# JiehongLin/SAM-6D

Hardware: AMD Instinct MI355X
Metric: RGB-D frames/sec (SAM-6D per-frame hot path: SAM ViT-H encoder + ISM scoring + PEM) (higher is better)
Workload: dtype bf16 (SAM ViT-H: 87 % of the step) + f16 (PEM ViT-B feature extractor) + f32 (ISM scoring, PEM point transformer and pose solvers); 1 GPU; LM-O single object: 32 frames/step/GPU, 640x480 RGB-D -> 1024^2 SAM input, P=128 proposals x 42 templates (scored in groups of 8 frames), 1 instance/frame, 2048 pts (PEM batch 32); sam_frames_per_launch_group=16, pem_vit_dtype=fp16 (set by bench.py; the library default is fp32)

## Files before the change

include/sam6d_hip.h:

```cpp
#ifndef SAM6D_HIP_H
#define SAM6D_HIP_H

#include <stdint.h>

#ifdef __cplusplus
extern "C" {
#endif

#define S6D_OK 0
#define S6D_EINVAL (-1)
#define S6D_ELAUNCH (-2)
#define S6D_EUNSUPPORTED (-3)

#define S6D_ABI_VERSION 135
int s6d_version(void);
int s6d_set_persistent_grid_limit(int max_workgroups);
int s6d_set_gemm_wave_tile(int columns);
int s6d_set_gemm_mfma_shape(int rows);
int s6d_set_gemm_small_tile(int enable);
const char *s6d_strerror(int code);
const char *s6d_last_hip_error(void);


int s6d_fps_f32(const float *xyz, int B, int N, int M, float *tmp, int32_t *idx, void *stream);

int s6d_gather_points_f32(const float *points, const int32_t *idx, int B, int C, int N, int M,
                          float *out, void *stream);

int s6d_ball_query_f32(const float *new_xyz, const float *xyz, int B, int N, int M, float radius,
                       int nsample, int32_t *idx, void *stream);

int s6d_group_points_f32(const float *points, const int32_t *idx, int B, int C, int N, int M, int S,
                         float *out, void *stream);

int s6d_gather_rows_f32(const float *src, const int32_t *idx, int B, int N, int C, int M, float *out,
                        void *stream);

int s6d_segment_seq_sum_f32(const float *x, const int64_t *start, const int64_t *count, int P, int C, float *out,
                            void *stream);

int s6d_pem_sample_indices_f32(const float *keys, long key_stride, const int64_t *count, int P, int n_sample,
                               int64_t *idx, int32_t *overflow, void *stream);

int s6d_pem_mask_boxes_u8(const unsigned char *mask, const float *depth, int P, int H, int W, long min_points,
                          unsigned char *m, int64_t *cnt, unsigned char *ok, int64_t *box, void *stream);

int s6d_pem_compact_cloud_f32(const unsigned char *m, const float *depth, const int64_t *box, const unsigned char *ok, int P,
                              int H, int W, float fx, float fy, float cx, float cy, long cap, int32_t *choose, float *cloud,
                              int64_t *n, void *stream);
int s6d_pem_radius_filter_f32(const float *center, const double *limit, int P, long cap, int32_t *choose, float *cloud,
                              int64_t *n, void *stream);

int s6d_pem_crops_f32(const unsigned char *image, const unsigned char *m, const int64_t *kept, const int64_t *box, int M,
                      int H, int W, int S, int use_mask, const float *mean3_host, const float *std3_host, float *out,
                      void *stream);


int s6d_template_boxes_u8(const unsigned char *mask, int T, int H, int W, int64_t *cnt, int64_t *box, int64_t *tight,
                          void *stream);

int s6d_template_points_f32(const unsigned char *mask, const float *xyz_mm, const int64_t *box, int T, int H, int W, long cap,
                            int32_t *choose, float *pts, int64_t *n, void *stream);

int s6d_template_pem_crops_f32(const unsigned char *images, const unsigned char *mask, const int64_t *box, int T, int H, int W,
                               int S, int use_mask, const float *mean3_host, const float *std3_host, float *out, void *stream);

int s6d_template_ism_crops_f32(const unsigned char *images, const unsigned char *mask, const void *params, int T, int H, int W,
// ... 29 lines not shown


int s6d_mask_pack_u8(const uint8_t *masks, int N, long HW, uint64_t *packed, int32_t *area, void *stream);

int s6d_mask_pair_inter(const uint64_t *dpacked, int Nd, const uint64_t *gpacked, int Ng, long words, const int32_t *pairs, int P,
                        int32_t *inter, void *stream);

int s6d_box_pair_iou_f64(const double *dboxes, int Nd, const double *gboxes, int Ng, const int32_t *pairs, int P, double *iou,
                         void *stream);

#define S6D_COCO_MATCH_MAX_GT 64
int s6d_coco_match(const double *ious, const long *iou_off, const int32_t *groups, const double *det_area, const double *gt_area,
                   const uint8_t *gt_ignore, const double *params, int n_groups, int NT, int NA, long n_det, long n_gt, long n_iou,
                   int32_t *match, uint8_t *ignore, void *stream);


int s6d_rot_from_h_f32(const float *H, int n, float *R, void *stream);

int s6d_weighted_procrustes_f32(const float *src, const float *ref, const float *weights, int B, int N, float weight_thresh,
                                float eps, float *R, float *t, void *stream);

int s6d_pose_hypotheses_f32(const float *pts1, const float *pts2, const int32_t *pair, int B, int N1,
                            int N2, int n_hyp, float *R, float *t, float *dis, void *stream);

int s6d_cosine_similarity_f32(const float *f1, const float *f2, int B, int M1, int M2, int C, float temp, float *atten, void *stream);

int s6d_coarse_sample_f32(const float *atten, const float *rand_u, int B, int M1, int M2, int n_u, int32_t *pair, float *w1,
                          void *stream);

int s6d_smallest_k_f32(const float *dis, const float *Rs, const float *ts, int B, int n, int k, float *Rk, float *tk,
                       int32_t *idx, void *stream);

int s6d_hypothesis_select_f32(const float *dmin, const float *w1, const float *Rk, const float *tk, int B, int P, int N,
                              float *R, float *t, void *stream);

int s6d_min_dist_f32(const float *pts, const float *R, const float *t, const float *model, int B, int N,
                     int P, int Nm, float *dmin, void *stream);


int s6d_rpe_attention_f32(const float *q, const float *k, const float *v, const float *qt, const float *qb,
                          const float *embed, int B, int N, int C, int heads, float scale, float *out,
                          void *stream);

int s6d_rpe_attention_packed_f32(const float *proj, long ld, int q_off, int k_off, int v_off, int qt_off, int qb_off,
                                 const float *embed, int B, int N, int C, int heads, float scale, float *out, void *stream);
int s6d_rpe_attention_packed_e16_f32(const float *proj, long ld, int q_off, int k_off, int v_off, int qt_off, int qb_off,
                                     const void *embed_f16, int B, int N, int C, int heads, float scale, float *out, void *stream);
int s6d_rpe_attention_strided_e16_f32(const float *q, long ldq, const float *k, long ldk, const float *v, long ldv, const float *qt,
                                      const float *qb, const void *embed_f16, int B, int N, int C, int heads, float scale, float *out,
                                      void *stream);
int s6d_rpe_attention_strided_f32(const float *q, long ldq, const float *k, long ldk, const float *v, long ldv, const float *qt,
                                  const float *qb, const float *embed, int B, int N, int C, int heads, float scale, float *out,
                                  void *stream);


int s6d_win_attention_bf16(const void *qkv, const void *qkv_bias, const void *rel_h, const void *rel_w, int B,
                           int H, int W, int num_heads, int head_dim, int window, float scale, void *rel_scratch,
                           void *out, void *stream);
int s6d_win_attention_layout_bf16(const void *qkv, int head_major, const void *qkv_bias, const void *rel_h, const void *rel_w,
                                  int B, int H, int W, int num_heads, int head_dim, int window, float scale,
                                  void *rel_scratch, void *out, void *stream);
int s6d_win_attention_pad_rel_bf16(const void *rel_h, const void *rel_w, int H, int window, int head_dim, void *rel_padded, void *stream);
int s6d_win_attention_prepadded_bf16(const void *qkv, int head_major, const void *qkv_bias, const void *rel_padded, int B, int H, int W,
                                     int num_heads, int head_dim, int window, float scale, void *out, void *stream);
long s6d_win_attention_scratch_bytes(int H, int window, int head_dim);

int s6d_add_layernorm_bf16(const void *x, const void *delta, const float *gamma, const float *beta, float eps,
                           long rows, int C, void *x_out, void *y_out, void *stream);
int s6d_layernorm_bf16_f32(const void *x, const float *gamma, const float *beta, float eps, long rows, int C, float *y_f32,
                           void *stream);

int s6d_gemm_bf16(const void *A, long lda, const void *W, long ldw, const float *bias, void *C, long ldc, int M, int N,
                  int K, int epilogue, int max_blocks, void *stream);
int s6d_gemm_bf16_cblk(const void *A, long lda, const void *W, long ldw, const float *bias, void *C, long ldc, int M, int N, int K,
                       int epilogue, int col_block, int max_blocks, void *stream);
int s6d_gemm_f16(const void *A, long lda, const void *W, long ldw, const float *bias, void *C, long ldc, int M, int N, int K,
                 int epilogue, int max_blocks, void *stream);
int s6d_add_layernorm_f16(const void *x, const void *delta, const float *gamma, const float *beta, float eps, long rows, int C,
                          void *x_out, void *y_out, void *stream);
int s6d_seq_attention_f16(const void *qkv, int B, int N, int num_heads, int head_dim, float scale, void *out, void *stream);
int s6d_seq_attention_strided_bf16(const void *qkv, long tok_stride, long which_stride, long head_stride, int B, int N,
                                   int num_heads, int head_dim, float scale, void *out, void *stream);
int s6d_seq_attention_strided_f16(const void *qkv, long tok_stride, long which_stride, long head_stride, int B, int N,
                                  int num_heads, int head_dim, float scale, void *out, void *stream);

int s6d_gemm_bf16_res(const void *A, long lda, const void *W, long ldw, const float *bias, const void *R, long ldr,
                      float *stats_partial, void *C, long ldc, int M, int N, int K, int max_blocks, void *stream);
int s6d_ln_stats_finalize(const float *stats_partial, int groups, int group_size, long M, float eps, float *row_stats, void *stream);
int s6d_row_stats_bf16(const void *x, long ldx, long M, int C, float eps, float *row_stats, void *stream);
int s6d_gemm_bf16_lnfold(const void *A, long lda, const float *row_stats, const void *W, long ldw, const float *col_sums,
                         const float *bias, void *C, long ldc, int M, int N, int K, int gelu, int col_block, int max_blocks,
                         void *stream);

int s6d_gemm_fp8(const void *A, long lda, const unsigned char *a_scale, const void *W, long ldw, const unsigned char *w_scale,
                 const float *bias, void *C, long ldc, int M, int N, int K, int epilogue, int max_blocks, void *stream);
int s6d_gemm_fp8_gelu_mx(const void *A, long lda, const unsigned char *a_scale, const void *W, long ldw, const unsigned char *w_scale,
                         const float *bias, void *C8, long ldc, unsigned char *c_scale, int M, int N, int K, int max_blocks,
                         void *stream);
int s6d_gemm_fp8_mxa(const void *A, long lda, const unsigned char *a_mx, const void *W, long ldw, const unsigned char *w_scale,
                     const float *bias, void *C, long ldc, int M, int N, int K, int epilogue, int max_blocks, void *stream);
int s6d_layernorm_fp8(const void *x, const float *gamma, const float *beta, float eps, long rows, int C, void *y8,
                      unsigned char *yscale, void *stream);
int s6d_add_layernorm_fp8(const void *x, const void *delta, const float *gamma, const float *beta, float eps, long rows, int C,
                          void *x_out, void *y8, unsigned char *yscale, void *stream);


// ... 176 lines not shown
```

sam6d_amd/csrc/s6d_rpe.hip:

```cpp
#include "s6d_common.h"
#include "s6d_mem.h"

namespace s6d {

__device__ __forceinline__ float dot4(const float4 a, const float4 b) {
  return __builtin_fmaf(a.w, b.w, __builtin_fmaf(a.z, b.z, __builtin_fmaf(a.y, b.y, a.x * b.x)));
}

template <int WAVES, bool RPE, bool EH = false, int KEYS = 4>
__global__ __launch_bounds__(WAVES * 64) void rpe_attention_kernel(
    const float *__restrict__ q, const float *__restrict__ k, const float *__restrict__ v,
    const float *__restrict__ qt, const float *__restrict__ qb, const void *__restrict__ embedv,
    int B, int N, int M, float scale, float *__restrict__ out, long ldq, long ldk, long ldv, long qt_bs, long qt_rs, long qt_hs,
    long qb_bs, long qb_rs, long qb_hs) {
  S6D_DYN_LDS(smem);
  const int wave = threadIdx.x >> 6, lane = threadIdx.x & 63;
  const int Np = (M + 3) & ~3;
  float *sc = reinterpret_cast<float *>(smem) + (size_t)wave * 4 * Np;
  const long row = (long)blockIdx.x * WAVES + wave;
  if (row >= (long)B * N) return;
  const int b = (int)(row / N), n = (int)(row % N);
  const int g = lane >> 4;
  const int c4 = lane * 4;

  const float4 q4 = *reinterpret_cast<const float4 *>(q + row * ldq + c4);
  float4 t0 = make_float4(0.f, 0.f, 0.f, 0.f), t1 = t0, t2 = t0, t3 = t0;
  float qbg = 0.f;
  const float *erow = nullptr;
  const _Float16 *erow_h = nullptr;
  if (RPE) {
    const float *base = qt + (size_t)b * qt_bs + (size_t)n * qt_rs + c4;
    t0 = *reinterpret_cast<const float4 *>(base);
    t1 = *reinterpret_cast<const float4 *>(base + qt_hs);
    t2 = *reinterpret_cast<const float4 *>(base + 2 * qt_hs);
    t3 = *reinterpret_cast<const float4 *>(base + 3 * qt_hs);
    qbg = qb[(size_t)b * qb_bs + (size_t)n * qb_rs + (size_t)g * qb_hs];
    if (EH) erow_h = reinterpret_cast<const _Float16 *>(embedv) + (size_t)row * M * 256 + c4;
    else erow = reinterpret_cast<const float *>(embedv) + (size_t)row * M * 256 + c4;
  }
  const float *krow = k + (size_t)b * M * ldk + c4;
  const float *vrow = v + (size_t)b * M * ldv + c4;
  const bool hi32 = lane & 32, hi16 = lane & 16;

  const bool hi8 = lane & 8, hi4 = lane & 4;
  for (int m0 = 0; m0 < M; m0 += KEYS) {
    float4 k4[KEYS], e4[KEYS];
#pragma unroll
    for (int u = 0; u < KEYS; ++u) {
      const int m = min(m0 + u, M - 1);
      k4[u] = *reinterpret_cast<const float4 *>(krow + (size_t)m * ldk);
      if (RPE) {
        if (EH) {
          typedef __attribute__((ext_vector_type(4))) _Float16 h4;
          const h4 e = *reinterpret_cast<const h4 *>(erow_h + (size_t)m * 256);
          e4[u] = make_float4((float)e[0], (float)e[1], (float)e[2], (float)e[3]);
        } else {
          e4[u] = *reinterpret_cast<const float4 *>(erow + (size_t)m * 256);
        }
      }
    }
    float mine[KEYS];
#pragma unroll
    for (int u = 0; u < KEYS; ++u) {
      mine[u] = 0.f;
      if (RPE) {
        const float p0 = dot4(t0, e4[u]), p1 = dot4(t1, e4[u]), p2 = dot4(t2, e4[u]), p3 = dot4(t3, e4[u]);
        float ka = hi32 ? p2 : p0, kb = hi32 ? p3 : p1;
        const float sa = hi32 ? p0 : p2, sb = hi32 ? p1 : p3;
        ka += __shfl_xor(sa, 32);
        kb += __shfl_xor(sb, 32);
        mine[u] = hi16 ? kb : ka;
        const float send = hi16 ? ka : kb;
        mine[u] += __shfl_xor(send, 16);
      }
      mine[u] += dot4(q4, k4[u]);
    }
    float s;
    int mu = m0;
    bool writer;
    if (KEYS == 4) {
      float a0 = hi8 ? mine[1] : mine[0], a1 = hi8 ? mine[KEYS - 1] : mine[KEYS / 2];
      a0 += __shfl_xor(hi8 ? mine[0] : mine[1], 8);
      a1 += __shfl_xor(hi8 ? mine[KEYS / 2] : mine[KEYS - 1], 8);
      s = hi4 ? a1 : a0;
      s += __shfl_xor(hi4 ? a0 : a1, 4);
      mu += ((lane >> 3) & 1) + 2 * ((lane >> 2) & 1);
      writer = (lane & 3) == 0;
    } else if (KEYS == 2) {
      s = hi8 ? mine[KEYS - 1] : mine[0];
      s += __shfl_xor(hi8 ? mine[0] : mine[KEYS - 1], 8);
      s += __shfl_xor(s, 4);
      mu += (lane >> 3) & 1;
      writer = (lane & 7) == 0;
    } else {
      s = mine[0];
      s += __shfl_xor(s, 8);
      s += __shfl_xor(s, 4);
      writer = (lane & 15) == 0;
    }
    s += __shfl_xor(s, 2);
    s += __shfl_xor(s, 1);
    if (writer && mu < M) sc[g * Np + mu] = (s + qbg) * scale;
  }
  __builtin_amdgcn_wave_barrier();
  float mx = -3.4e38f;
  for (int m = lane & 15; m < M; m += 16) mx = fmaxf(mx, sc[g * Np + m]);
  mx = fmaxf(mx, __shfl_xor(mx, 8));
  mx = fmaxf(mx, __shfl_xor(mx, 4));
  mx = fmaxf(mx, __shfl_xor(mx, 2));
  mx = fmaxf(mx, __shfl_xor(mx, 1));
  float sum = 0.f;
  for (int m = lane & 15; m < M; m += 16) {
    const float e = __expf(sc[g * Np + m] - mx);
    sc[g * Np + m] = e;
    sum += e;
  }
  sum += __shfl_xor(sum, 8);
  sum += __shfl_xor(sum, 4);
  sum += __shfl_xor(sum, 2);
  sum += __shfl_xor(sum, 1);
  const float inv = 1.0f / sum;
  __builtin_amdgcn_wave_barrier();
  float4 acc = make_float4(0.f, 0.f, 0.f, 0.f);
  for (int m = 0; m < M; ++m) {
    const float a = sc[g * Np + m];
    const float4 v4 = *reinterpret_cast<const float4 *>(vrow + (size_t)m * ldv);
    acc.x = __builtin_fmaf(a, v4.x, acc.x); acc.y = __builtin_fmaf(a, v4.y, acc.y);
    acc.z = __builtin_fmaf(a, v4.z, acc.z); acc.w = __builtin_fmaf(a, v4.w, acc.w);
  }
  acc.x *= inv; acc.y *= inv; acc.z *= inv; acc.w *= inv;
  *reinterpret_cast<float4 *>(out + row * 256 + c4) = acc;
}

}

using namespace s6d;

#ifndef S6D_RPE_KEYS_FULL
#define S6D_RPE_KEYS_FULL 1
#endif
#ifndef S6D_RPE_FOUR_KEYS_MAX_ROWS
#define S6D_RPE_FOUR_KEYS_MAX_ROWS 5000
#endif
static inline int rpe_keys(long rows) { return rows <= S6D_RPE_FOUR_KEYS_MAX_ROWS ? 4 : S6D_RPE_KEYS_FULL; }
#define S6D_RPE_LAUNCH(EHV, KEYSV, GRID, LDS, ST, ...)                                                              \
  do {                                                                                                            \
    if ((KEYSV) == 4) hipLaunchKernelGGL((rpe_attention_kernel<4, true, EHV, 4>), GRID, dim3(256), LDS, ST, __VA_ARGS__);      \
    else if ((KEYSV) == 2) hipLaunchKernelGGL((rpe_attention_kernel<4, true, EHV, 2>), GRID, dim3(256), LDS, ST, __VA_ARGS__); \
    else hipLaunchKernelGGL((rpe_attention_kernel<4, true, EHV, 1>), GRID, dim3(256), LDS, ST, __VA_ARGS__);                   \
  } while (0)

static int rpe_strided(const float *q, long ldq, const float *k, long ldk, const float *v, long ldv, const float *qt, const float *qb,
                       const void *embed, bool eh, int B, int N, int C, int heads, float scale, float *out, void *stream) {
  if (B < 0 || N <= 0 || ldq < C || ldk < C || ldv < C || (ldq % 4) || (ldk % 4) || (ldv % 4)) return S6D_EINVAL;
  if (C != 256 || heads != 4) return S6D_EUNSUPPORTED;
  if (B == 0) return S6D_OK;
  if (!q || !k || !v || !qt || !qb || !embed || !out) return S6D_EINVAL;
  if (((uintptr_t)q | (uintptr_t)k | (uintptr_t)v) & 15) return S6D_EINVAL;
  constexpr int WAVES = 4;
  const long rows = (long)B * N;
  const int Np = (N + 3) & ~3;
  const size_t lds = (size_t)WAVES * 4 * Np * sizeof(float);
  if (lds > 64 * 1024) return S6D_EUNSUPPORTED;
  static_assert(WAVES == 4, "S6D_RPE_LAUNCH instantiates the four-wave kernels");
  const dim3 grid((unsigned)((rows + WAVES - 1) / WAVES));
  const int keys = rpe_keys(rows);
  if (eh)
    S6D_RPE_LAUNCH(true, keys, grid, lds, as_stream(stream), q, k, v, qt, qb, embed, B, N, N, scale, out, ldq, ldk, ldv, 4L * N * 256,
                   256L, (long)N * 256, 4L * N, 1L, (long)N);
  else
    S6D_RPE_LAUNCH(false, keys, grid, lds, as_stream(stream), q, k, v, qt, qb, embed, B, N, N, scale, out, ldq, ldk, ldv, 4L * N * 256,
                   256L, (long)N * 256, 4L * N, 1L, (long)N);
  return launch_status();
}

extern "C" int s6d_rpe_attention_strided_f32(const float *q, long ldq, const float *k, long ldk, const float *v, long ldv,
                                             const float *qt, const float *qb, const float *embed, int B, int N, int C, int heads,
                                             float scale, float *out, void *stream) {
  return rpe_strided(q, ldq, k, ldk, v, ldv, qt, qb, embed, false, B, N, C, heads, scale, out, stream);
}

extern "C" int s6d_rpe_attention_strided_e16_f32(const float *q, long ldq, const float *k, long ldk, const float *v, long ldv,
                                                 const float *qt, const float *qb, const void *embed_f16, int B, int N, int C, int heads,
                                                 float scale, float *out, void *stream) {
  return rpe_strided(q, ldq, k, ldk, v, ldv, qt, qb, embed_f16, true, B, N, C, heads, scale, out, stream);
}

static int rpe_packed(const float *proj, long ld, int q_off, int k_off, int v_off, int qt_off, int qb_off, const void *embed, bool eh,
                      int B, int N, int C, int heads, float scale, float *out, void *stream) {
  if (B < 0 || N <= 0 || C != 256 || heads != 4 || (ld % 4) != 0) return B < 0 || N <= 0 || (ld % 4) ? S6D_EINVAL : S6D_EUNSUPPORTED;
  if (q_off < 0 || k_off < 0 || v_off < 0 || qt_off < 0 || qb_off < 0 || (q_off % 4) || (k_off % 4) || (v_off % 4) || (qt_off % 4) ||
      q_off + C > ld || k_off + C > ld || v_off + C > ld || qt_off + 4 * C > ld || qb_off + 4 > ld)
    return S6D_EINVAL;
  if (B == 0) return S6D_OK;
  if (!proj || !embed || !out || ((uintptr_t)proj & 15)) return S6D_EINVAL;
  constexpr int WAVES = 4;
  const long rows = (long)B * N;
  const int Np = (N + 3) & ~3;
  const size_t lds = (size_t)WAVES * 4 * Np * sizeof(float);
  if (lds > 64 * 1024) return S6D_EUNSUPPORTED;
  static_assert(WAVES == 4, "S6D_RPE_LAUNCH instantiates the four-wave kernels");
  const dim3 grid((unsigned)((rows + WAVES - 1) / WAVES));
  const int keys = rpe_keys(rows);
  if (eh)
    S6D_RPE_LAUNCH(true, keys, grid, lds, as_stream(stream), proj + q_off, proj + k_off, proj + v_off, proj + qt_off, proj + qb_off,
                   embed, B, N, N, scale, out, ld, ld, ld, (long)N * ld, ld, 256L, (long)N * ld, ld, 1L);
  else
    S6D_RPE_LAUNCH(false, keys, grid, lds, as_stream(stream), proj + q_off, proj + k_off, proj + v_off, proj + qt_off, proj + qb_off,
                   embed, B, N, N, scale, out, ld, ld, ld, (long)N * ld, ld, 256L, (long)N * ld, ld, 1L);
  return launch_status();
}

extern "C" int s6d_rpe_attention_packed_f32(const float *proj, long ld, int q_off, int k_off, int v_off, int qt_off, int qb_off,
                                            const float *embed, int B, int N, int C, int heads, float scale, float *out,
                                            void *stream) {
  return rpe_packed(proj, ld, q_off, k_off, v_off, qt_off, qb_off, embed, false, B, N, C, heads, scale, out, stream);
}

extern "C" int s6d_rpe_attention_packed_e16_f32(const float *proj, long ld, int q_off, int k_off, int v_off, int qt_off, int qb_off,
                                                const void *embed_f16, int B, int N, int C, int heads, float scale, float *out,
                                                void *stream) {
  return rpe_packed(proj, ld, q_off, k_off, v_off, qt_off, qb_off, embed_f16, true, B, N, C, heads, scale, out, stream);
}

extern "C" int s6d_rpe_attention_f32(const float *q, const float *k, const float *v, const float *qt,
                                     const float *qb, const float *embed, int B, int N, int C, int heads,
                                     float scale, float *out, void *stream) {
  return s6d_rpe_attention_strided_f32(q, C, k, C, v, C, qt, qb, embed, B, N, C, heads, scale, out, stream);
}

extern "C" int s6d_mha_strided_f32(const float *q, long ldq, const float *k, long ldk, const float *v, long ldv, int B, int N, int M,
                                   int C, int heads, float scale, float *out, void *stream) {
  if (B < 0 || N <= 0 || M <= 0 || ldq < C || ldk < C || ldv < C || (ldq % 4) || (ldk % 4) || (ldv % 4)) return S6D_EINVAL;
  if (C != 256 || heads != 4) return S6D_EUNSUPPORTED;
  if (B == 0) return S6D_OK;
  if (!q || !k || !v || !out) return S6D_EINVAL;
  if (((uintptr_t)q | (uintptr_t)k | (uintptr_t)v) & 15) return S6D_EINVAL;
  constexpr int WAVES = 4;
  const long rows = (long)B * N;
  const int Np = (M + 3) & ~3;
  const size_t lds = (size_t)WAVES * 4 * Np * sizeof(float);
  if (lds > 64 * 1024) return S6D_EUNSUPPORTED;
  hipLaunchKernelGGL((rpe_attention_kernel<WAVES, false, false, 4>), dim3((unsigned)((rows + WAVES - 1) / WAVES)), dim3(WAVES * 64),
                     lds, as_stream(stream), q, k, v, nullptr, nullptr, nullptr, B, N, M, scale, out, ldq, ldk, ldv, 0L, 0L, 0L, 0L, 0L, 0L);
  return launch_status();
}

extern "C" int s6d_mha_f32(const float *q, const float *k, const float *v, int B, int N, int M, int C, int heads,
                           float scale, float *out, void *stream) {
  return s6d_mha_strided_f32(q, C, k, C, v, C, B, N, M, C, heads, scale, out, stream);
}

__global__ __launch_bounds__(256) void focus_kernel(const float *__restrict__ x, const float *__restrict__ inv_scale,
                                                    long rows, int p, float *__restrict__ y) {
  const long row = (long)blockIdx.x * 4 + (threadIdx.x >> 6);
  if (row >= rows) return;
  const int lane = threadIdx.x & 63;
  const float4 a = *reinterpret_cast<const float4 *>(x + row * 256 + lane * 4);
  const float4 is = *reinterpret_cast<const float4 *>(inv_scale + lane * 4);
  float t[4] = {(fmaxf(a.x, 0.f) + 1e-6f) * is.x, (fmaxf(a.y, 0.f) + 1e-6f) * is.y, (fmaxf(a.z, 0.f) + 1e-6f) * is.z,
                (fmaxf(a.w, 0.f) + 1e-6f) * is.w};
  float n1 = t[0] * t[0] + t[1] * t[1] + t[2] * t[2] + t[3] * t[3];
  float u[4];
#pragma unroll
  for (int e = 0; e < 4; ++e) {
    float r = t[e];
    for (int i = 1; i < p; ++i) r *= t[e];
    u[e] = r;
  }
  float n3 = u[0] * u[0] + u[1] * u[1] + u[2] * u[2] + u[3] * u[3];
  n1 = wave_sum(n1);
  n3 = wave_sum(n3);
  const float f = sqrtf(n1) / sqrtf(n3);
  *reinterpret_cast<float4 *>(y + row * 256 + lane * 4) = make_float4(u[0] * f, u[1] * f, u[2] * f, u[3] * f);
}

extern "C" int s6d_linear_attn_focus_f32(const float *x, const float *inv_scale, long rows, int C, int power, float *y,
                                         void *stream) {
  if (rows < 0 || power < 1) return S6D_EINVAL;
  if (C != 256) return S6D_EUNSUPPORTED;
  if (rows == 0) return S6D_OK;
  if (!x || !inv_scale || !y) return S6D_EINVAL;
  hipLaunchKernelGGL(focus_kernel, dim3((unsigned)((rows + 3) / 4)), dim3(256), 0, as_stream(stream), x, inv_scale, rows,
                     power, y);
  return launch_status();
}
```

sam6d_amd/ops.py:

```python
import ctypes

import torch

from . import _lib
from . import policy


def _stream():
    return torch.cuda.current_stream().cuda_stream


def _ptr(t):
    return None if t is None else t.data_ptr()


def _float3(values):
    return (ctypes.c_float * 3)(*[float(v) for v in values])


def _chk(t, dtype, name, ndim=None):
    if not t.is_cuda:
        raise RuntimeError(f"{name} must be a CUDA tensor")
    if not t.is_contiguous():
        raise RuntimeError(f"{name} must be a contiguous tensor")
# ... 120 lines not shown
def coarse_sample(atten, rand_u):
    _chk(atten, torch.float32, "atten", 3)
    _chk(rand_u, torch.float32, "rand_u", 2)
    B, M1, M2 = atten.shape
    pair = torch.empty(B, rand_u.shape[1], dtype=torch.int32, device=atten.device)
    w1 = torch.empty(B, M1 - 1, dtype=torch.float32, device=atten.device)
    _call("s6d_coarse_sample_f32", _ptr(atten), _ptr(rand_u), B, M1, M2, rand_u.shape[1], _ptr(pair), _ptr(w1), _stream())
    return pair, w1


def smallest_k(dis, Rs, ts, k):
    _chk(dis, torch.float32, "dis", 2)
    _chk(Rs, torch.float32, "Rs", 4)
    _chk(ts, torch.float32, "ts", 3)
    B, n = dis.shape
    Rk = torch.empty(B, k, 3, 3, dtype=torch.float32, device=dis.device)
    tk = torch.empty(B, k, 3, dtype=torch.float32, device=dis.device)
    idx = torch.empty(B, k, dtype=torch.int32, device=dis.device)
    _call("s6d_smallest_k_f32", _ptr(dis), _ptr(Rs), _ptr(ts), B, n, k, _ptr(Rk), _ptr(tk), _ptr(idx), _stream())
    return Rk, tk, idx


def hypothesis_select(dmin, w1, Rk, tk):
    for a, nm, nd in ((dmin, "dmin", 3), (w1, "w1", 2), (Rk, "Rk", 4), (tk, "tk", 3)):
        _chk(a, torch.float32, nm, nd)
    B, P, N = dmin.shape
    R = torch.empty(B, 3, 3, dtype=torch.float32, device=dmin.device)
    t = torch.empty(B, 3, dtype=torch.float32, device=dmin.device)
    _call("s6d_hypothesis_select_f32", _ptr(dmin), _ptr(w1), _ptr(Rk), _ptr(tk), B, P, N, _ptr(R), _ptr(t), _stream())
    return R, t


def min_dist(pts, R, t, model):
    for a, nm, nd in ((pts, "pts", 3), (R, "R", 4), (t, "t", 3), (model, "model", 3)):
        _chk(a, torch.float32, nm, nd)
    B, N, _ = pts.shape
    P, Nm = R.shape[1], model.shape[1]
    out = torch.empty(B, P, N, dtype=torch.float32, device=pts.device)
    _call("s6d_min_dist_f32", _ptr(pts), _ptr(R), _ptr(t), _ptr(model), B, N, P, Nm, _ptr(out), _stream())
    return out


def _rows3(t, name):
    if not t.is_cuda or t.dtype != torch.float32 or t.dim() != 3:
        raise RuntimeError(f"{name} must be a 3-d float32 CUDA tensor")
    B, N, C = t.shape
    if t.stride(2) == 1 and t.stride(1) % 4 == 0 and t.stride(1) >= C and (B == 1 or t.stride(0) == N * t.stride(1)) \
            and t.data_ptr() % 16 == 0:
        return t, t.stride(1)
    t = t.contiguous()
    return t, C


ATTN_ROWS_MAX_KEYS = 1024


def rpe_attention(q, k, v, qt, qb, embed, scale):
    (q, ldq), (k, ldk), (v, ldv) = _rows3(q, "q"), _rows3(k, "k"), _rows3(v, "v")
    qt, qb = qt.contiguous(), qb.contiguous()
    for a, nm in ((qt, "qt"), (qb, "qb")):
        _chk(a, torch.float32, nm)
    _chk(embed, embed.dtype if embed.dtype == torch.float16 else torch.float32, "embed", 4)
    B, N, C = q.shape
    out = torch.empty(B, N, C, dtype=torch.float32, device=q.device)
    _call("s6d_rpe_attention_strided_e16_f32" if embed.dtype == torch.float16 else "s6d_rpe_attention_strided_f32", _ptr(q), ldq, _ptr(k),
          ldk, _ptr(v), ldv, _ptr(qt), _ptr(qb), _ptr(embed), B, N, C, 4, scale, _ptr(out), _stream())
    return out


def rpe_attention_packed(proj, embed, scale, q_off=0, k_off=256, v_off=512, qt_off=768, qb_off=1792):
    _chk(proj, torch.float32, "proj", 3)
    _chk(embed, embed.dtype if embed.dtype == torch.float16 else torch.float32, "embed", 4)
    B, N, ld = proj.shape
    out = torch.empty(B, N, 256, dtype=torch.float32, device=proj.device)
    _call("s6d_rpe_attention_packed_e16_f32" if embed.dtype == torch.float16 else "s6d_rpe_attention_packed_f32", _ptr(proj), ld,
          int(q_off), int(k_off), int(v_off), int(qt_off), int(qb_off), _ptr(embed), B, N, 256, 4, scale, _ptr(out), _stream())
    return out


def sam_preprocess(x, mean, std, img_size, out_dtype=torch.bfloat16):
    _chk(x, torch.float32, "x", 4)
    B, C, h, w = x.shape
    if C != 3:
        raise RuntimeError("x must have 3 channels")
    out = torch.empty(B, 3, img_size, img_size, dtype=out_dtype, device=x.device)
    _call("s6d_sam_preprocess_f32", _ptr(x), B, h, w, int(img_size), _float3(mean), _float3(std), 1 if out_dtype == torch.bfloat16 else 0,
          _ptr(out), _stream())
    return out


def nonfinite_rows(x):
    _chk(x, torch.float32, "x")
    B = x.shape[0]
    n = x.numel() // max(B, 1)
    flags = torch.empty(B, dtype=torch.int32, device=x.device)
    _call("s6d_nonfinite_rows_f32", _ptr(x), B, n, _ptr(flags), _stream())
    return flags.bool()


def im2col3x3(y):
    if y.dtype not in (torch.bfloat16, torch.float16) or y.dim() != 4 or not y.is_contiguous():
        raise RuntimeError("im2col3x3: contiguous (B,H,W,C) bf16 / f16 expected")
    B, H, W, C = y.shape
    out = torch.empty(B, H, W, 9 * C, dtype=y.dtype, device=y.device)
    _call("s6d_im2col3x3_b16", _ptr(y), B, H, W, C, _ptr(out), _stream())
    return out

# ... 864 lines not shown
    if w.dim() != 2 or w.shape[1] != K or w.stride(1) != 1 or w.stride(0) % 8:
        raise RuntimeError("w must be (N, K) with contiguous rows")
    if bias is not None:
        _chk(bias, torch.float32, "bias", 1)
    M = a2.shape[0]
    if col_block:
        if out is not None:
            raise RuntimeError("col_block output is allocated by the call")
        out = torch.empty(N // col_block, M, col_block, dtype=torch.bfloat16, device=a.device)
        _call("s6d_gemm_bf16_cblk", _ptr(a2), a2.stride(0), _ptr(w), w.stride(0), _ptr(bias), _ptr(out), N, M, N, K, 1 if gelu else 0,
              int(col_block), int(max_blocks), _stream())
        return out
    if out is None:
        out = torch.empty(M, N, dtype=a.dtype, device=a.device)
    else:
        _chk(out, a.dtype, "out", 2)
        if tuple(out.shape) != (M, N) or out.stride(1) != 1 or out.stride(0) % 8 or out.data_ptr() % 16:
            raise ValueError(f"out must be ({M}, {N}) bf16 with contiguous, 16-byte aligned rows (stride % 8 == 0); got "
                             f"{tuple(out.shape)} strides {tuple(out.stride())}")
    rows = gemm_one_launch_rows(a2.stride(0))
    if residual is not None:
        if gelu or col_block:
            raise RuntimeError("the residual form takes neither GELU nor column blocks")
        _chk(residual, torch.bfloat16, "residual")
        r2 = residual.reshape(-1, N)
        if r2.shape[0] != M:
            raise ValueError(f"residual has {r2.shape[0]} rows, the product {M}")
        if r2.stride(1) != 1 or r2.stride(0) % 8 or r2.data_ptr() % 16:
            raise ValueError("residual rows must be contiguous and 16-byte aligned")
        if stats_partial is not None:
            _chk(stats_partial, torch.float32, "stats_partial")
            if tuple(stats_partial.shape) != (N // 32, 2, M) or not stats_partial.is_contiguous():
                raise ValueError(f"stats_partial must be a contiguous ({N // 32}, 2, {M}) f32 tensor; got {tuple(stats_partial.shape)}")
            if M > rows:
                raise RuntimeError("row statistics are written for one launch: the row count exceeds one 2-GiB slab")
        for r0 in range(0, M, rows):
            r1 = min(M, r0 + rows)
            _call("s6d_gemm_bf16_res", _ptr(a2[r0:r1]), a2.stride(0), _ptr(w), w.stride(0), _ptr(bias), _ptr(r2[r0:r1]), r2.stride(0),
                  _ptr(stats_partial), _ptr(out[r0:r1]), out.stride(0), r1 - r0, N, K, int(max_blocks), _stream())
        return out.reshape(*a.shape[:-1], N)
    if stats_partial is not None:
        raise RuntimeError("stats_partial comes with the residual form")
    for r0 in range(0, M, rows):
        r1 = min(M, r0 + rows)
        _call("s6d_gemm_f16" if f16 else "s6d_gemm_bf16", _ptr(a2[r0:r1]), a2.stride(0), _ptr(w), w.stride(0), _ptr(bias), _ptr(out[r0:r1]),
              out.stride(0), r1 - r0, N, K, 1 if gelu else 0, int(max_blocks), _stream())
    return out.reshape(*a.shape[:-1], N)


def set_geo_embed_form(form):
    _call("s6d_set_geo_embed_form", int(form))


def set_gemm_small_tile(enable):
    _call("s6d_set_gemm_small_tile", int(enable))


def set_gemm_wave_tile(columns):
    _call("s6d_set_gemm_wave_tile", int(columns))


def set_gemm_mfma_shape(rows):
    _call("s6d_set_gemm_mfma_shape", int(rows))


def gemm_one_launch_rows(row_stride, elem_bytes=2):
    return max(256, ((2 ** 31 - 1) // (elem_bytes * int(row_stride))) // 256 * 256)


def ln_stats_finalize(stats_partial, group_size=32, eps=1e-6):
    _chk(stats_partial, torch.float32, "stats_partial", 3)
    if not stats_partial.is_contiguous() or stats_partial.shape[1] != 2:
        raise ValueError("stats_partial must be a contiguous (groups, 2, M) tensor")
    G, _, M = stats_partial.shape
    out = torch.empty(M, 2, dtype=torch.float32, device=stats_partial.device)
    _call("s6d_ln_stats_finalize", _ptr(stats_partial), G, int(group_size), M, eps, _ptr(out), _stream())
    return out


def row_stats(x, eps=1e-6):
    _chk(x, torch.bfloat16, "x")
    C = x.shape[-1]
    x2 = x.reshape(-1, C)
    if x2.stride(1) != 1 or x2.stride(0) % 8 or x2.data_ptr() % 16:
        x2 = x2.contiguous()
    out = torch.empty(x2.shape[0], 2, dtype=torch.float32, device=x.device)
    _call("s6d_row_stats_bf16", _ptr(x2), x2.stride(0), x2.shape[0], C, eps, _ptr(out), _stream())
    return out


def gemm_bf16_lnfold(a, stats, w_folded, col_sums, bias, gelu=False, col_block=0, max_blocks=0):
    _chk(a, torch.bfloat16, "a")
    _chk(w_folded, torch.bfloat16, "w_folded", 2)
    _chk(stats, torch.float32, "stats", 2)
    _chk(col_sums, torch.float32, "col_sums", 1)
    _chk(bias, torch.float32, "bias", 1)
    K, N = a.shape[-1], w_folded.shape[0]
    a2 = a.reshape(-1, K)
    if a2.stride(1) != 1 or a2.stride(0) % 8 or a2.data_ptr() % 16:
        a2 = a2.contiguous()
    M = a2.shape[0]
    if w_folded.shape[1] != K or w_folded.stride(1) != 1 or w_folded.stride(0) % 8:
        raise RuntimeError("w_folded must be (N, K) with contiguous rows")
    if tuple(stats.shape) != (M, 2) or not stats.is_contiguous() or col_sums.numel() != N or bias.numel() != N:
        raise ValueError(f"stats must be ({M}, 2), col_sums and bias ({N},)")
    if M > gemm_one_launch_rows(a2.stride(0)):
# ... 455 lines not shown
```

Measured before the change: 168.3 frames/s.

## Share K/V rows across waves via double-buffered LDS staging in row attention

Adds a shared-staging variant of the per-row attention kernel in which the waves of a workgroup (query rows of the same batch) cooperatively load chunks of 8 K and V rows into double-buffered LDS and read them from there. Each wave no longer fetches every key/value row from global memory on its own, which is meant to cut redundant global traffic in the PEM point-transformer attention. This variant becomes the default, with 8 waves per workgroup for the non-RPE path. The change adds block-wide barriers per chunk and more LDS, so the score-buffer limit drops to 48 KiB and ATTN_ROWS_MAX_KEYS falls from 1024 to 768, sending larger key counts to another path.

After: 169.2 frames/s (median of 6 runs). No clear change (+0.5%).

```diff
diff --git a/include/sam6d_hip.h b/include/sam6d_hip.h
--- a/include/sam6d_hip.h
+++ b/include/sam6d_hip.h
@@ -12,7 +12,7 @@
 #define S6D_ELAUNCH (-2)
 #define S6D_EUNSUPPORTED (-3)
 
-#define S6D_ABI_VERSION 135
+#define S6D_ABI_VERSION 136
 int s6d_version(void);
 int s6d_set_persistent_grid_limit(int max_workgroups);
 int s6d_set_gemm_wave_tile(int columns);
@@ -148,6 +148,7 @@
 int s6d_rpe_attention_strided_f32(const float *q, long ldq, const float *k, long ldk, const float *v, long ldv, const float *qt,
                                   const float *qb, const float *embed, int B, int N, int C, int heads, float scale, float *out,
                                   void *stream);
+int s6d_set_rpe_attention_form(int shared_rows, int keys);
 
 
 int s6d_win_attention_bf16(const void *qkv, const void *qkv_bias, const void *rel_h, const void *rel_w, int B,
diff --git a/sam6d_amd/csrc/s6d_rpe.hip b/sam6d_amd/csrc/s6d_rpe.hip
--- a/sam6d_amd/csrc/s6d_rpe.hip
+++ b/sam6d_amd/csrc/s6d_rpe.hip
@@ -5,6 +5,98 @@
 
 __device__ __forceinline__ float dot4(const float4 a, const float4 b) {
   return __builtin_fmaf(a.w, b.w, __builtin_fmaf(a.z, b.z, __builtin_fmaf(a.y, b.y, a.x * b.x)));
+}
+
+
+template <bool RPE, bool EH, int KEYS>
+__device__ __forceinline__ void rows_load_embed(float4 (&e4)[KEYS], const float *erow, const _Float16 *erow_h, int m0, int M) {
+#pragma unroll
+  for (int u = 0; u < KEYS; ++u) {
+    const int m = min(m0 + u, M - 1);
+    if (RPE) {
+      if (EH) {
+        typedef __attribute__((ext_vector_type(4))) _Float16 h4;
+        const h4 e = *reinterpret_cast<const h4 *>(erow_h + (size_t)m * 256);
+        e4[u] = make_float4((float)e[0], (float)e[1], (float)e[2], (float)e[3]);
+      } else {
+        e4[u] = *reinterpret_cast<const float4 *>(erow + (size_t)m * 256);
+      }
+    }
+  }
+}
+
+template <bool RPE, int KEYS>
+__device__ __forceinline__ void rows_score_trip(const float4 (&k4)[KEYS], const float4 (&e4)[KEYS], const float4 q4, const float4 t0,
+                                                const float4 t1, const float4 t2, const float4 t3, float qbg, float scale, float *scg,
+                                                int m0, int M, int lane) {
+  const bool hi32 = lane & 32, hi16 = lane & 16, hi8 = lane & 8, hi4 = lane & 4;
+  float mine[KEYS];
+#pragma unroll
+  for (int u = 0; u < KEYS; ++u) {
+    mine[u] = 0.f;
+    if (RPE) {
+      const float p0 = dot4(t0, e4[u]), p1 = dot4(t1, e4[u]), p2 = dot4(t2, e4[u]), p3 = dot4(t3, e4[u]);
+      float ka = hi32 ? p2 : p0, kb = hi32 ? p3 : p1;
+      const float sa = hi32 ? p0 : p2, sb = hi32 ? p1 : p3;
+      ka += __shfl_xor(sa, 32);
+      kb += __shfl_xor(sb, 32);
+      mine[u] = hi16 ? kb : ka;
+      const float send = hi16 ? ka : kb;
+      mine[u] += __shfl_xor(send, 16);
+    }
+    mine[u] += dot4(q4, k4[u]);
+  }
+  float s;
+  int mu = m0;
+  bool writer;
+  if (KEYS == 4) {
+    float a0 = hi8 ? mine[1] : mine[0], a1 = hi8 ? mine[KEYS - 1] : mine[KEYS / 2];
+    a0 += __shfl_xor(hi8 ? mine[0] : mine[1], 8);
+    a1 += __shfl_xor(hi8 ? mine[KEYS / 2] : mine[KEYS - 1], 8);
+    s = hi4 ? a1 : a0;
+    s += __shfl_xor(hi4 ? a0 : a1, 4);
+    mu += ((lane >> 3) & 1) + 2 * ((lane >> 2) & 1);
+    writer = (lane & 3) == 0;
+  } else if (KEYS == 2) {
+    s = hi8 ? mine[KEYS - 1] : mine[0];
+    s += __shfl_xor(hi8 ? mine[0] : mine[KEYS - 1], 8);
+    s += __shfl_xor(s, 4);
+    mu += (lane >> 3) & 1;
+    writer = (lane & 7) == 0;
+  } else {
+    s = mine[0];
+    s += __shfl_xor(s, 8);
+    s += __shfl_xor(s, 4);
+    writer = (lane & 15) == 0;
+  }
+  s += __shfl_xor(s, 2);
+  s += __shfl_xor(s, 1);
+  if (writer && mu < M) scg[mu] = (s + qbg) * scale;
+}
+
+__device__ __forceinline__ float rows_softmax(float *scg, int M, int lane) {
+  float mx = -3.4e38f;
+  for (int m = lane & 15; m < M; m += 16) mx = fmaxf(mx, scg[m]);
+  mx = fmaxf(mx, __shfl_xor(mx, 8));
+  mx = fmaxf(mx, __shfl_xor(mx, 4));
+  mx = fmaxf(mx, __shfl_xor(mx, 2));
+  mx = fmaxf(mx, __shfl_xor(mx, 1));
+  float sum = 0.f;
+  for (int m = lane & 15; m < M; m += 16) {
+    const float e = __expf(scg[m] - mx);
+    scg[m] = e;
+    sum += e;
+  }
+  sum += __shfl_xor(sum, 8);
+  sum += __shfl_xor(sum, 4);
+  sum += __shfl_xor(sum, 2);
+  sum += __shfl_xor(sum, 1);
+  return 1.0f / sum;
+}
+
+__device__ __forceinline__ void rows_pv_step(float4 &acc, float a, const float4 v4) {
+  acc.x = __builtin_fmaf(a, v4.x, acc.x); acc.y = __builtin_fmaf(a, v4.y, acc.y);
+  acc.z = __builtin_fmaf(a, v4.z, acc.z); acc.w = __builtin_fmaf(a, v4.w, acc.w);
 }
 
 template <int WAVES, bool RPE, bool EH = false, int KEYS = 4>
@@ -40,96 +132,128 @@
   }
   const float *krow = k + (size_t)b * M * ldk + c4;
   const float *vrow = v + (size_t)b * M * ldv + c4;
-  const bool hi32 = lane & 32, hi16 = lane & 16;
-
-  const bool hi8 = lane & 8, hi4 = lane & 4;
+  float *scg = sc + g * Np;
+
   for (int m0 = 0; m0 < M; m0 += KEYS) {
     float4 k4[KEYS], e4[KEYS];
 #pragma unroll
-    for (int u = 0; u < KEYS; ++u) {
-      const int m = min(m0 + u, M - 1);
-      k4[u] = *reinterpret_cast<const float4 *>(krow + (size_t)m * ldk);
-      if (RPE) {
-        if (EH) {
-          typedef __attribute__((ext_vector_type(4))) _Float16 h4;
-          const h4 e = *reinterpret_cast<const h4 *>(erow_h + (size_t)m * 256);
-          e4[u] = make_float4((float)e[0], (float)e[1], (float)e[2], (float)e[3]);
-        } else {
-          e4[u] = *reinterpret_cast<const float4 *>(erow + (size_t)m * 256);
-        }
+    for (int u = 0; u < KEYS; ++u) k4[u] = *reinterpret_cast<const float4 *>(krow + (size_t)min(m0 + u, M - 1) * ldk);
+    rows_load_embed<RPE, EH, KEYS>(e4, erow, erow_h, m0, M);
+    rows_score_trip<RPE, KEYS>(k4, e4, q4, t0, t1, t2, t3, qbg, scale, scg, m0, M, lane);
+  }
+  __builtin_amdgcn_wave_barrier();
+  const float inv = rows_softmax(scg, M, lane);
+  __builtin_amdgcn_wave_barrier();
+  float4 acc = make_float4(0.f, 0.f, 0.f, 0.f);
+  for (int m = 0; m < M; ++m) rows_pv_step(acc, scg[m], *reinterpret_cast<const float4 *>(vrow + (size_t)m * ldv));
+  acc.x *= inv; acc.y *= inv; acc.z *= inv; acc.w *= inv;
+  *reinterpret_cast<float4 *>(out + row * 256 + c4) = acc;
+}
+
+constexpr int RPE_CHUNK = 8;
+constexpr int RPE_STAGE_BYTES = 2 * RPE_CHUNK * 256 * (int)sizeof(float);
+
+template <int WAVES>
+__device__ __forceinline__ void rows_stage_fetch(float4 &st0, float4 &st1, const float *base, long ld, int m0, int M, int wave) {
+  st0 = *reinterpret_cast<const float4 *>(base + (size_t)min(m0 + wave, M - 1) * ld);
+  if (WAVES < RPE_CHUNK) st1 = *reinterpret_cast<const float4 *>(base + (size_t)min(m0 + wave + WAVES, M - 1) * ld);
+}
+template <int WAVES>
+__device__ __forceinline__ void rows_stage_put(const float4 st0, const float4 st1, float *buf, int wave, int c4) {
+  *reinterpret_cast<float4 *>(buf + wave * 256 + c4) = st0;
+  if (WAVES < RPE_CHUNK) *reinterpret_cast<float4 *>(buf + (wave + WAVES) * 256 + c4) = st1;
+}
+
+template <int WAVES, bool RPE, bool EH = false, int KEYS = 4>
+__global__ __launch_bounds__(WAVES * 64) void rpe_attention_shared_kernel(
+    const float *__restrict__ q, const float *__restrict__ k, const float *__restrict__ v,
+    const float *__restrict__ qt, const float *__restrict__ qb, const void *__restrict__ embedv,
+    int B, int N, int M, float scale, float *__restrict__ out, long ldq, long ldk, long ldv, long qt_bs, long qt_rs, long qt_hs,
+    long qb_bs, long qb_rs, long qb_hs) {
+  static_assert((RPE_CHUNK == WAVES || RPE_CHUNK == 2 * WAVES) && RPE_CHUNK % KEYS == 0, "one or two rows of a chunk per wave, whole trips");
+  S6D_DYN_LDS(smem);
+  const int wave = threadIdx.x >> 6, lane = threadIdx.x & 63;
+  const int Np = (M + 3) & ~3;
+  float *scg = reinterpret_cast<float *>(smem) + ((size_t)wave * 4 + (lane >> 4)) * Np;
+  float *stage = reinterpret_cast<float *>(smem) + (size_t)WAVES * 4 * Np;
+  const int groups = (N + WAVES - 1) / WAVES;
+  const int b = blockIdx.x / groups, nw = (blockIdx.x % groups) * WAVES + wave;
+  const bool live = nw < N;
+  const int n = live ? nw : N - 1;
+  const long row = (long)b * N + n;
+  const int c4 = lane * 4;
+
+  const float4 q4 = *reinterpret_cast<const float4 *>(q + row * ldq + c4);
+  float4 t0 = make_float4(0.f, 0.f, 0.f, 0.f), t1 = t0, t2 = t0, t3 = t0;
+  float qbg = 0.f;
+  const float *erow = nullptr;
+  const _Float16 *erow_h = nullptr;
+  if (RPE) {
+    const float *base = qt + (size_t)b * qt_bs + (size_t)n * qt_rs + c4;
+    t0 = *reinterpret_cast<const float4 *>(base);
+    t1 = *reinterpret_cast<const float4 *>(base + qt_hs);
+    t2 = *reinterpret_cast<const float4 *>(base + 2 * qt_hs);
+    t3 = *reinterpret_cast<const float4 *>(base + 3 * qt_hs);
+    qbg = qb[(size_t)b * qb_bs + (size_t)n * qb_rs + (size_t)(lane >> 4) * qb_hs];
+    if (EH) erow_h = reinterpret_cast<const _Float16 *>(embedv) + (size_t)row * M * 256 + c4;
+    else erow = reinterpret_cast<const float *>(embedv) + (size_t)row * M * 256 + c4;
+  }
+  const float *krow = k + (size_t)b * M * ldk + c4;
+  const float *vrow = v + (size_t)b * M * ldv + c4;
+
+  float4 st0, st1 = make_float4(0.f, 0.f, 0.f, 0.f);
+  const int chunks = (M + RPE_CHUNK - 1) / RPE_CHUNK;
+
+  rows_stage_fetch<WAVES>(st0, st1, krow, ldk, 0, M, wave);
+  rows_stage_put<WAVES>(st0, st1, stage, wave, c4);
+  __syncthreads();
+  for (int c = 0; c < chunks; ++c) {
+    const int m0 = c * RPE_CHUNK;
+    const bool more = c + 1 < chunks;
+    if (more) rows_stage_fetch<WAVES>(st0, st1, krow, ldk, m0 + RPE_CHUNK, M, wave);
+    const float *kst = stage + (size_t)(c & 1) * RPE_CHUNK * 256 + c4;
+    if (m0 + RPE_CHUNK <= M) {
+#pragma unroll
+      for (int j = 0; j < RPE_CHUNK; j += KEYS) {
+        float4 k4[KEYS], e4[KEYS];
+        rows_load_embed<RPE, EH, KEYS>(e4, erow, erow_h, m0 + j, M);
+#pragma unroll
+        for (int u = 0; u < KEYS; ++u) k4[u] = *reinterpret_cast<const float4 *>(kst + (j + u) * 256);
+        rows_score_trip<RPE, KEYS>(k4, e4, q4, t0, t1, t2, t3, qbg, scale, scg, m0 + j, M, lane);
+      }
+    } else {
+      for (int j = 0; m0 + j < M; j += KEYS) {
+        float4 k4[KEYS], e4[KEYS];
+        rows_load_embed<RPE, EH, KEYS>(e4, erow, erow_h, m0 + j, M);
+#pragma unroll
+        for (int u = 0; u < KEYS; ++u) k4[u] = *reinterpret_cast<const float4 *>(kst + (j + u) * 256);
+        rows_score_trip<RPE, KEYS>(k4, e4, q4, t0, t1, t2, t3, qbg, scale, scg, m0 + j, M, lane);
       }
     }
-    float mine[KEYS];
-#pragma unroll
-    for (int u = 0; u < KEYS; ++u) {
-      mine[u] = 0.f;
-      if (RPE) {
-        const float p0 = dot4(t0, e4[u]), p1 = dot4(t1, e4[u]), p2 = dot4(t2, e4[u]), p3 = dot4(t3, e4[u]);
-        float ka = hi32 ? p2 : p0, kb = hi32 ? p3 : p1;
-        const float sa = hi32 ? p0 : p2, sb = hi32 ? p1 : p3;
-        ka += __shfl_xor(sa, 32);
-        kb += __shfl_xor(sb, 32);
-        mine[u] = hi16 ? kb : ka;
-        const float send = hi16 ? ka : kb;
-        mine[u] += __shfl_xor(send, 16);
-      }
-      mine[u] += dot4(q4, k4[u]);
+    if (more) rows_stage_put<WAVES>(st0, st1, stage + ((c + 1) & 1) * RPE_CHUNK * 256, wave, c4);
+    __syncthreads();
+  }
+  rows_stage_fetch<WAVES>(st0, st1, vrow, ldv, 0, M, wave);
+  const float inv = rows_softmax(scg, M, lane);
+  rows_stage_put<WAVES>(st0, st1, stage, wave, c4);
+  __syncthreads();
+  float4 acc = make_float4(0.f, 0.f, 0.f, 0.f);
+  for (int c = 0; c < chunks; ++c) {
+    const int m0 = c * RPE_CHUNK;
+    const bool more = c + 1 < chunks;
+    if (more) rows_stage_fetch<WAVES>(st0, st1, vrow, ldv, m0 + RPE_CHUNK, M, wave);
+    const float *vst = stage + (size_t)(c & 1) * RPE_CHUNK * 256 + c4;
+    if (m0 + RPE_CHUNK <= M) {
+#pragma unroll
+      for (int j = 0; j < RPE_CHUNK; ++j) rows_pv_step(acc, scg[m0 + j], *reinterpret_cast<const float4 *>(vst + j * 256));
+    } else {
+      for (int j = 0; m0 + j < M; ++j) rows_pv_step(acc, scg[m0 + j], *reinterpret_cast<const float4 *>(vst + j * 256));
     }
-    float s;
-    int mu = m0;
-    bool writer;
-    if (KEYS == 4) {
-      float a0 = hi8 ? mine[1] : mine[0], a1 = hi8 ? mine[KEYS - 1] : mine[KEYS / 2];
-      a0 += __shfl_xor(hi8 ? mine[0] : mine[1], 8);
-      a1 += __shfl_xor(hi8 ? mine[KEYS / 2] : mine[KEYS - 1], 8);
-      s = hi4 ? a1 : a0;
-      s += __shfl_xor(hi4 ? a0 : a1, 4);
-      mu += ((lane >> 3) & 1) + 2 * ((lane >> 2) & 1);
-      writer = (lane & 3) == 0;
-    } else if (KEYS == 2) {
-      s = hi8 ? mine[KEYS - 1] : mine[0];
-      s += __shfl_xor(hi8 ? mine[0] : mine[KEYS - 1], 8);
-      s += __shfl_xor(s, 4);
-      mu += (lane >> 3) & 1;
-      writer = (lane & 7) == 0;
-    } else {
-      s = mine[0];
-      s += __shfl_xor(s, 8);
-      s += __shfl_xor(s, 4);
-      writer = (lane & 15) == 0;
-    }
-    s += __shfl_xor(s, 2);
-    s += __shfl_xor(s, 1);
-    if (writer && mu < M) sc[g * Np + mu] = (s + qbg) * scale;
-  }
-  __builtin_amdgcn_wave_barrier();
-  float mx = -3.4e38f;
-  for (int m = lane & 15; m < M; m += 16) mx = fmaxf(mx, sc[g * Np + m]);
-  mx = fmaxf(mx, __shfl_xor(mx, 8));
-  mx = fmaxf(mx, __shfl_xor(mx, 4));
-  mx = fmaxf(mx, __shfl_xor(mx, 2));
-  mx = fmaxf(mx, __shfl_xor(mx, 1));
-  float sum = 0.f;
-  for (int m = lane & 15; m < M; m += 16) {
-    const float e = __expf(sc[g * Np + m] - mx);
-    sc[g * Np + m] = e;
-    sum += e;
-  }
-  sum += __shfl_xor(sum, 8);
-  sum += __shfl_xor(sum, 4);
-  sum += __shfl_xor(sum, 2);
-  sum += __shfl_xor(sum, 1);
-  const float inv = 1.0f / sum;
-  __builtin_amdgcn_wave_barrier();
-  float4 acc = make_float4(0.f, 0.f, 0.f, 0.f);
-  for (int m = 0; m < M; ++m) {
-    const float a = sc[g * Np + m];
-    const float4 v4 = *reinterpret_cast<const float4 *>(vrow + (size_t)m * ldv);
-    acc.x = __builtin_fmaf(a, v4.x, acc.x); acc.y = __builtin_fmaf(a, v4.y, acc.y);
-    acc.z = __builtin_fmaf(a, v4.z, acc.z); acc.w = __builtin_fmaf(a, v4.w, acc.w);
+    if (more) rows_stage_put<WAVES>(st0, st1, stage + ((c + 1) & 1) * RPE_CHUNK * 256, wave, c4);
+    __syncthreads();
   }
   acc.x *= inv; acc.y *= inv; acc.z *= inv; acc.w *= inv;
-  *reinterpret_cast<float4 *>(out + row * 256 + c4) = acc;
+  if (live) *reinterpret_cast<float4 *>(out + row * 256 + c4) = acc;
 }
 
 }
@@ -142,13 +266,59 @@
 #ifndef S6D_RPE_FOUR_KEYS_MAX_ROWS
 #define S6D_RPE_FOUR_KEYS_MAX_ROWS 5000
 #endif
-static inline int rpe_keys(long rows) { return rows <= S6D_RPE_FOUR_KEYS_MAX_ROWS ? 4 : S6D_RPE_KEYS_FULL; }
-#define S6D_RPE_LAUNCH(EHV, KEYSV, GRID, LDS, ST, ...)                                                              \
-  do {                                                                                                            \
-    if ((KEYSV) == 4) hipLaunchKernelGGL((rpe_attention_kernel<4, true, EHV, 4>), GRID, dim3(256), LDS, ST, __VA_ARGS__);      \
-    else if ((KEYSV) == 2) hipLaunchKernelGGL((rpe_attention_kernel<4, true, EHV, 2>), GRID, dim3(256), LDS, ST, __VA_ARGS__); \
-    else hipLaunchKernelGGL((rpe_attention_kernel<4, true, EHV, 1>), GRID, dim3(256), LDS, ST, __VA_ARGS__);                   \
-  } while (0)
+static inline int rpe_keys(long rows, int shared_rows) {
+  return shared_rows != 1 || rows <= S6D_RPE_FOUR_KEYS_MAX_ROWS ? 4 : S6D_RPE_KEYS_FULL;
+}
+static int g_rpe_shared_rows = 0, g_rpe_keys = 0;
+extern "C" int s6d_set_rpe_attention_form(int shared_rows, int keys) {
+  if ((shared_rows != 0 && shared_rows != 1 && shared_rows != 4 && shared_rows != 8) || (keys != 0 && keys != 1 && keys != 2 && keys != 4))
+    return S6D_EINVAL;
+  g_rpe_shared_rows = shared_rows;
+  g_rpe_keys = keys;
+  return S6D_OK;
+}
+
+static_assert(48 * 1024 + RPE_STAGE_BYTES == 64 * 1024, "the launchers' `lds > 48 * 1024` is the score part of the 64 KiB budget");
+
+struct RowsOperands {
+  const float *q, *k, *v, *qt, *qb;
+  const void *embed;
+  int B, N, M;
+  float scale;
+  float *out;
+  long ldq, ldk, ldv, qt_bs, qt_rs, qt_hs, qb_bs, qb_rs, qb_hs;
+};
+
+template <bool RPE, bool EH, int KEYS>
+static int rows_launch_keys(int shared_rows, const RowsOperands &a, void *stream) {
+  const size_t wave_scores = (size_t)4 * ((a.M + 3) & ~3) * sizeof(float);
+  const unsigned groups4 = (unsigned)((a.N + 3) / 4), groups8 = (unsigned)((a.N + 7) / 8);
+#define S6D_ROWS_ARGS a.q, a.k, a.v, a.qt, a.qb, a.embed, a.B, a.N, a.M, a.scale, a.out, a.ldq, a.ldk, a.ldv, a.qt_bs, a.qt_rs, a.qt_hs, \
+                      a.qb_bs, a.qb_rs, a.qb_hs
+  if (shared_rows == 1) {
+    hipLaunchKernelGGL((rpe_attention_kernel<4, RPE, EH, KEYS>), dim3((unsigned)(((long)a.B * a.N + 3) / 4)), dim3(256), 4 * wave_scores,
+                       as_stream(stream), S6D_ROWS_ARGS);
+  } else if (shared_rows == 4) {
+    hipLaunchKernelGGL((rpe_attention_shared_kernel<4, RPE, EH, KEYS>), dim3((unsigned)a.B * groups4), dim3(256),
+                       4 * wave_scores + RPE_STAGE_BYTES, as_stream(stream), S6D_ROWS_ARGS);
+  } else {
+    if (8 * wave_scores + RPE_STAGE_BYTES > 64 * 1024) return S6D_EUNSUPPORTED;
+    hipLaunchKernelGGL((rpe_attention_shared_kernel<8, RPE, EH, KEYS>), dim3((unsigned)a.B * groups8), dim3(512),
+                       8 * wave_scores + RPE_STAGE_BYTES, as_stream(stream), S6D_ROWS_ARGS);
+  }
+#undef S6D_ROWS_ARGS
+  return launch_status();
+}
+
+template <bool RPE, bool EH>
+static int rows_launch(const RowsOperands &a, void *stream) {
+  const bool eight_fit = (size_t)8 * 4 * ((a.M + 3) & ~3) * sizeof(float) + RPE_STAGE_BYTES <= 64 * 1024;
+  const int shared_rows = g_rpe_shared_rows ? g_rpe_shared_rows : (!RPE && eight_fit ? 8 : 4);
+  const int keys = g_rpe_keys ? g_rpe_keys : (RPE ? rpe_keys((long)a.B * a.N, shared_rows) : 4);
+  if (keys == 4) return rows_launch_keys<RPE, EH, 4>(shared_rows, a, stream);
+  if (keys == 2) return rows_launch_keys<RPE, EH, 2>(shared_rows, a, stream);
+  return rows_launch_keys<RPE, EH, 1>(shared_rows, a, stream);
+}
 
 static int rpe_strided(const float *q, long ldq, const float *k, long ldk, const float *v, long ldv, const float *qt, const float *qb,
                        const void *embed, bool eh, int B, int N, int C, int heads, float scale, float *out, void *stream) {
@@ -158,20 +328,11 @@
   if (!q || !k || !v || !qt || !qb || !embed || !out) return S6D_EINVAL;
   if (((uintptr_t)q | (uintptr_t)k | (uintptr_t)v) & 15) return S6D_EINVAL;
   constexpr int WAVES = 4;
-  const long rows = (long)B * N;
   const int Np = (N + 3) & ~3;
   const size_t lds = (size_t)WAVES * 4 * Np * sizeof(float);
-  if (lds > 64 * 1024) return S6D_EUNSUPPORTED;
-  static_assert(WAVES == 4, "S6D_RPE_LAUNCH instantiates the four-wave kernels");
-  const dim3 grid((unsigned)((rows + WAVES - 1) / WAVES));
-  const int keys = rpe_keys(rows);
-  if (eh)
-    S6D_RPE_LAUNCH(true, keys, grid, lds, as_stream(stream), q, k, v, qt, qb, embed, B, N, N, scale, out, ldq, ldk, ldv, 4L * N * 256,
-                   256L, (long)N * 256, 4L * N, 1L, (long)N);
-  else
-    S6D_RPE_LAUNCH(false, keys, grid, lds, as_stream(stream), q, k, v, qt, qb, embed, B, N, N, scale, out, ldq, ldk, ldv, 4L * N * 256,
-                   256L, (long)N * 256, 4L * N, 1L, (long)N);
-  return launch_status();
+  if (lds > 48 * 1024) return S6D_EUNSUPPORTED;
+  const RowsOperands a = {q, k, v, qt, qb, embed, B, N, N, scale, out, ldq, ldk, ldv, 4L * N * 256, 256L, (long)N * 256, 4L * N, 1L, (long)N};
+  return eh ? rows_launch<true, true>(a, stream) : rows_launch<true, false>(a, stream);
 }
 
 extern "C" int s6d_rpe_attention_strided_f32(const float *q, long ldq, const float *k, long ldk, const float *v, long ldv,
@@ -195,20 +356,12 @@
   if (B == 0) return S6D_OK;
   if (!proj || !embed || !out || ((uintptr_t)proj & 15)) return S6D_EINVAL;
   constexpr int WAVES = 4;
-  const long rows = (long)B * N;
   const int Np = (N + 3) & ~3;
   const size_t lds = (size_t)WAVES * 4 * Np * sizeof(float);
-  if (lds > 64 * 1024) return S6D_EUNSUPPORTED;
-  static_assert(WAVES == 4, "S6D_RPE_LAUNCH instantiates the four-wave kernels");
-  const dim3 grid((unsigned)((rows + WAVES - 1) / WAVES));
-  const int keys = rpe_keys(rows);
-  if (eh)
-    S6D_RPE_LAUNCH(true, keys, grid, lds, as_stream(stream), proj + q_off, proj + k_off, proj + v_off, proj + qt_off, proj + qb_off,
-                   embed, B, N, N, scale, out, ld, ld, ld, (long)N * ld, ld, 256L, (long)N * ld, ld, 1L);
-  else
-    S6D_RPE_LAUNCH(false, keys, grid, lds, as_stream(stream), proj + q_off, proj + k_off, proj + v_off, proj + qt_off, proj + qb_off,
-                   embed, B, N, N, scale, out, ld, ld, ld, (long)N * ld, ld, 256L, (long)N * ld, ld, 1L);
-  return launch_status();
+  if (lds > 48 * 1024) return S6D_EUNSUPPORTED;
+  const RowsOperands a = {proj + q_off, proj + k_off, proj + v_off, proj + qt_off, proj + qb_off, embed, B, N, N, scale, out, ld, ld, ld,
+                          (long)N * ld, ld, 256L, (long)N * ld, ld, 1L};
+  return eh ? rows_launch<true, true>(a, stream) : rows_launch<true, false>(a, stream);
 }
 
 extern "C" int s6d_rpe_attention_packed_f32(const float *proj, long ld, int q_off, int k_off, int v_off, int qt_off, int qb_off,
@@ -237,13 +390,11 @@
   if (!q || !k || !v || !out) return S6D_EINVAL;
   if (((uintptr_t)q | (uintptr_t)k | (uintptr_t)v) & 15) return S6D_EINVAL;
   constexpr int WAVES = 4;
-  const long rows = (long)B * N;
   const int Np = (M + 3) & ~3;
   const size_t lds = (size_t)WAVES * 4 * Np * sizeof(float);
-  if (lds > 64 * 1024) return S6D_EUNSUPPORTED;
-  hipLaunchKernelGGL((rpe_attention_kernel<WAVES, false, false, 4>), dim3((unsigned)((rows + WAVES - 1) / WAVES)), dim3(WAVES * 64),
-                     lds, as_stream(stream), q, k, v, nullptr, nullptr, nullptr, B, N, M, scale, out, ldq, ldk, ldv, 0L, 0L, 0L, 0L, 0L, 0L);
-  return launch_status();
+  if (lds > 48 * 1024) return S6D_EUNSUPPORTED;
+  const RowsOperands a = {q, k, v, nullptr, nullptr, nullptr, B, N, M, scale, out, ldq, ldk, ldv, 0L, 0L, 0L, 0L, 0L, 0L};
+  return rows_launch<false, false>(a, stream);
 }
 
 extern "C" int s6d_mha_f32(const float *q, const float *k, const float *v, int B, int N, int M, int C, int heads,
diff --git a/sam6d_amd/ops.py b/sam6d_amd/ops.py
--- a/sam6d_amd/ops.py
+++ b/sam6d_amd/ops.py
@@ -196,7 +196,7 @@
     return t, C
 
 
-ATTN_ROWS_MAX_KEYS = 1024
+ATTN_ROWS_MAX_KEYS = 768
 
 
 def rpe_attention(q, k, v, qt, qb, embed, scale):
@@ -1167,6 +1167,10 @@
     _call("s6d_set_geo_embed_form", int(form))
 
 
+def set_rpe_attention_form(shared_rows, keys=0):
+    _call("s6d_set_rpe_attention_form", int(shared_rows), int(keys))
+
+
 def set_gemm_small_tile(enable):
     _call("s6d_set_gemm_small_tile", int(enable))
 
```
